# hyye/lio-mapping

Measured on AMD Instinct MI355X. Metric: sliding-window solves/sec, 64-line 130k-pt scans, window=15 (opt_window=5), higher is better.
Workload: dtype f64 (solve) / f32 (features); 1 GPU; HDL-64E outdoor_test_config_64, S_outdoor ray-cast scans, window_size=15 opt_window_size=5, one SolveOptimization per step, clouds resident in HBM; n_lidar_residuals=78236, local_map_points=76752, surf_stack_points=19386, parallelism=1 window

## Files before the change

### lio-mapping_amd/csrc/capi.hip

```cpp
#include <cstring>
#include <new>

#include "../../include/lio_c.h"
#include "../../include/lio_test_hooks.h"
#include "../../include/lio_ext.h"
#include "../../include/lio_full_cloud.h"
#include "../../include/lio_odom_batch.h"
#include "../../include/lio_frontend_batch.h"
#include "../../include/lio_map_batch.h"
#include "est_batch.h"
#include "seg_sort.h"
#include "estimator.h"
#include "rccl_comm.h"
#include "host_init.h"
#include "kf_batch.h"
#include <mutex>
#include <thread>
#include <atomic>
#include <algorithm>

#include "mapping.h"
#include "odometry.h"
#include "pointproc.h"

using namespace lio;

struct lio_pim { std::shared_ptr<Preintegration> p; };
struct lio_map { std::unique_ptr<MappingDev> m; bool borrowed = false; };
struct lio_est { std::unique_ptr<Estimator> e; EstConfig cfg; lio_map map; lio_map_config map_cfg; std::unique_ptr<EstimatorBatch> solo; bool adopted = false; struct lio_est_batch *owner = nullptr; };
struct lio_est_batch {
  std::unique_ptr<EstimatorBatch> b, b2;
  int n1 = 0;
  int parts_opt = 0;
  std::vector<std::pair<std::string, int>> options;
  std::vector<lio_est *> members;
};
static constexpr int kBatchSplitFrom = 96;
struct lio_pp_pool { PointProcessorDev pp; std::mutex mu; unsigned long gen = 0; lio_pp_pool(float lo, float up, int r, const lio_pp_config &c) : pp(lo, up, r, c) {} };
struct lio_pp { std::unique_ptr<PointProcessorDev> pp; std::shared_ptr<lio_pp_pool> pool; int pool_sweep = -1; unsigned long pool_gen = 0; };
struct lio_odom { std::unique_ptr<OdometryDev> o; };

static V3d v3(const double *p) { return V3d(p[0], p[1], p[2]); }
// ... 550 lines not shown
  DBuf<int32_t> idx;
  DBuf<float> sqd, nbr;
  DBuf<float> bounds;
  DBuf<double> gn_partials, gn_sums;
  DBuf<OdomState> gn_state;
  DBuf<KfDesc> gn_kd;
  DBuf<float> gn_rows;
};
static Scratch &scratch() {
  static thread_local Scratch sc;
  if (!sc.s) {
    int nd = 0;
    LIO_HIP(hipGetDeviceCount(&nd));
    if (nd <= 0) throw DeviceError("no HIP device: the product has no CPU path");
    LIO_HIP(hipStreamCreate(&sc.s));
  }
  return sc;
}

int lio_voxel_grid(const float *xyzi, size_t n, float leaf, float *out, size_t *n_out) {
  if ((!xyzi && n) || !out || !n_out || !(leaf > 0)) return LIO_ERR_ARG;
  return guarded([&] {
    Scratch &sc = scratch();
    sc.a.reserve(std::max<size_t>(n, 1));
    if (n) LIO_HIP(hipMemcpyAsync(sc.a.p, xyzi, n * sizeof(float4), hipMemcpyHostToDevice, sc.s));
    size_t m = sc.vox.run(sc.a.p, n, leaf, sc.b, sc.s);
    if (m) LIO_HIP(hipMemcpyAsync(out, sc.b.p, m * sizeof(float4), hipMemcpyDeviceToHost, sc.s));
    LIO_HIP(hipStreamSynchronize(sc.s));
    *n_out = m;
    return LIO_OK;
  });
}

int lio_knn(const float *map, size_t n_map, const float *query, size_t m, int k, float radius_sq, int32_t *idx, float *sqd) {
  if ((!map && n_map) || (!query && m) || !(k == 1 || k == 5) || !idx || !sqd) return LIO_ERR_ARG;
  if (!(radius_sq > 0)) return LIO_ERR_ARG;
  if (m > size_t(INT_MAX) / 8 || n_map > size_t(INT_MAX)) return LIO_ERR_CAPACITY;
  return guarded([&] {
    Scratch &sc = scratch();
    sc.a.reserve(std::max<size_t>(n_map, 1)); sc.b.reserve(std::max<size_t>(m, 1));
    sc.idx.reserve(std::max<size_t>(m * k, 1)); sc.sqd.reserve(std::max<size_t>(m * k, 1));
    if (n_map) LIO_HIP(hipMemcpyAsync(sc.a.p, map, n_map * sizeof(float4), hipMemcpyHostToDevice, sc.s));
    if (m) LIO_HIP(hipMemcpyAsync(sc.b.p, query, m * sizeof(float4), hipMemcpyHostToDevice, sc.s));
    float mn[3], mx[3];
    host_cloud_bounds(map, n_map, mn, mx);
    sc.grid.build(sc.a.p, n_map, mn, mx, knn_cell_edge(radius_sq), sc.s);
    launch_knn(sc.b.p, int(m), k, radius_sq, sc.grid.sorted(), sc.grid.cells(), sc.grid.desc(), sc.idx.p, sc.sqd.p, sc.s);
    if (m) {
      LIO_HIP(hipMemcpyAsync(idx, sc.idx.p, m * k * sizeof(int32_t), hipMemcpyDeviceToHost, sc.s));
      LIO_HIP(hipMemcpyAsync(sqd, sc.sqd.p, m * k * sizeof(float), hipMemcpyDeviceToHost, sc.s));
    }
    LIO_HIP(hipStreamSynchronize(sc.s));
    return LIO_OK;
  });
}

int lio_knn_walk(const float *map, size_t n_map, const float *query, size_t m, float cell, int lanes_per_query, int32_t *idx, float *sqd,
                 float *nbr_xyz) {
  if ((!map && n_map) || (!query && m) || !idx || !sqd || !nbr_xyz || !(cell > 0) || !std::isfinite(cell)) return LIO_ERR_ARG;
  if (!(lanes_per_query == 1 || lanes_per_query == 4 || lanes_per_query == 8)) return LIO_ERR_ARG;
  if (m > size_t(INT_MAX) / 8 || n_map > size_t(INT_MAX)) return LIO_ERR_CAPACITY;
  return guarded([&] {
    Scratch &sc = scratch();
    sc.a.reserve(std::max<size_t>(n_map, 1)); sc.b.reserve(std::max<size_t>(m, 1));
    sc.idx.reserve(std::max<size_t>(m * 5, 1)); sc.sqd.reserve(std::max<size_t>(m * 5, 1)); sc.nbr.reserve(std::max<size_t>(m * 15, 1));
    if (n_map) LIO_HIP(hipMemcpyAsync(sc.a.p, map, n_map * sizeof(float4), hipMemcpyHostToDevice, sc.s));
// ... 920 lines not shown
```

### lio-mapping_amd/csrc/cloud_device.h

```cpp
#pragma once
#include <hip/hip_runtime.h>

#include <cfloat>
#include <climits>

#include "cloud_kernels.h"
#include "hmath.h"

#if defined(__HIPCC__)
namespace lio {

__device__ inline bool finite3(const float4 &p) { return isfinite(p.x) && isfinite(p.y) && isfinite(p.z); }
__device__ inline bool finite3(const Vec3<float> &p) { return isfinite(p.x) && isfinite(p.y) && isfinite(p.z); }


template <bool NORMALISE_CONJ>
__device__ __forceinline__ float4 to_end_point(float4 p, float s, const Quat<float> &qe, const Vec3<float> &te) {
  p.x -= s * te.x; p.y -= s * te.y; p.z -= s * te.z;
  Quat<float> qid;
  Quat<float> qs = slerp(qid, s, qe, FLT_EPSILON);
  Quat<float> qc = conj(qs);
  if (NORMALISE_CONJ) qc = normalized(qc);
  Vec3<float> v = rotate(qc, Vec3<float>(p.x, p.y, p.z));
  v = rotate(qe, v);
// ... 147 lines not shown
                                                     const int *__restrict__ tile_heads, int n, int tile, float4 *__restrict__ out) {
  __shared__ float4 sp[VOX_TILE];
  __shared__ uint32_t sk[VOX_TILE];
  __shared__ int swave[VOX_TILE / 64], sbase[VOX_TILE / 64];
  const int tid = threadIdx.x, lane = tid & 63, wv = tid >> 6;
  const int base_i = tile * VOX_TILE, i = base_i + tid;
  int before = 0;
  for (int b = tid; b < tile; b += VOX_TILE) before += tile_heads[b];
#pragma unroll
  for (int o = 32; o > 0; o >>= 1) before += __shfl_xor(before, o, 64);
  const uint32_t k = i < n ? keys[i] : VOX_KEY_NONE;
  sk[tid] = k;
  if (k != VOX_KEY_NONE) sp[tid] = pts[vals[i]];
  const bool head = vox_is_head(keys, i, k);
  const unsigned long long hb = __ballot(head);
  if (lane == 0) { swave[wv] = __popcll(hb); sbase[wv] = before; }
  __syncthreads();
  int pos = (sbase[0] + sbase[1]) + (sbase[2] + sbase[3]);
  for (int w = 0; w < wv; ++w) pos += swave[w];
  pos += __popcll(hb & ((1ull << lane) - 1ull));
  if (head) {
    float ax = 0, ay = 0, az = 0, ai = 0;
    int e = tid;
    while (e < VOX_TILE && sk[e] == k) { const float4 p = sp[e]; ax += p.x; ay += p.y; az += p.z; ai += p.w; ++e; }
    int cnt = e - tid;
    if (e == VOX_TILE) {
      int g = base_i + VOX_TILE;
      while (g < n && keys[g] == k) { const float4 p = pts[vals[g]]; ax += p.x; ay += p.y; az += p.z; ai += p.w; ++g; ++cnt; }
    }
    const float c = float(cnt);
    out[pos] = make_float4(ax / c, ay / c, az / c, ai / c);
  }
  return VoxSlot{pos, head};
}

__device__ __forceinline__ void clear_valid_block(uint8_t *__restrict__ valid, size_t n) {
  const size_t i = (size_t(blockIdx.x) * VOX_TILE + threadIdx.x) * 16;
  if (i + 16 <= n) *reinterpret_cast<uint4 *>(valid + i) = make_uint4(0, 0, 0, 0);
  else for (size_t k = i; k < n; ++k) valid[k] = 0;
}
__device__ __forceinline__ void odom_state_init(OdomState *__restrict__ st, const float *__restrict__ T, bool converged) {
  static_assert(offsetof(OdomState, T) == 0 && sizeof(OdomState) <= VOX_TILE * 4, "state layout: T first, the rest zero");
  unsigned *o = reinterpret_cast<unsigned *>(st);
  const int nw = int(sizeof(OdomState) / 4);
  if (int(threadIdx.x) < nw) {
    unsigned v = threadIdx.x < 8 ? __float_as_uint(T[threadIdx.x]) : 0u;
    if (converged && threadIdx.x == offsetof(OdomState, converged) / 4) v = 1u;
    o[threadIdx.x] = v;
  }
}


#define FEAT_LPQ 8
#ifndef KNN_BATCH
#define KNN_BATCH 4
#endif
__device__ __forceinline__ unsigned long long knn_key(float d, int idx) {
  return (static_cast<unsigned long long>(__float_as_uint(d)) << 32) | static_cast<unsigned int>(idx);
}
template <int K>
__device__ __forceinline__ void knn_insert(unsigned long long key, int j, unsigned long long (&bk)[K], int (&bj)[K]) {
  if (key < bk[K - 1]) {
    bk[K - 1] = key; bj[K - 1] = j;
#pragma unroll
    for (int k = K - 1; k > 0; --k) {
      const bool sw = bk[k - 1] > bk[k];
// ... 452 lines not shown
```

### lio-mapping_amd/csrc/cloud_kernels.h

```cpp
#pragma once
#include <cmath>
#include <cstdint>

#include "dev.h"
#include "hmath.h"

namespace lio {

struct VoxParams {
  float mn[3], mx[3];
  int minb[3], divb[3];
  int overflow;
  int n_valid;
};

struct Affine3f { float m[12]; };

#define LIO_MAX_FRAMES 32

struct ConcatSeg { const float4 *src; int n; int dst_off; int set_intensity; float intensity; Affine3f tf; int identity; };
struct ConcatArgs { ConcatSeg seg[LIO_MAX_FRAMES]; int nseg; int total; };
void launch_transform_concat(const ConcatArgs &a, float4 *dst, hipStream_t s);

void launch_deskew_to_end(float4 *pts, int n, const float q[4], const float p[3], float time_factor, hipStream_t s, bool keep_intensity = false);
void launch_rigid_map(const float4 *in, int n, const float q[4], const float p[3], float4 *out, hipStream_t s);

void launch_cloud_bounds(const float4 *pts, int n, DBuf<float> &partial, VoxParams *d_out, hipStream_t s);

class VoxelGridDev {
 public:
  size_t run(const float4 *in, size_t n, float leaf, DBuf<float4> &out, hipStream_t s, VoxParams *host_params = nullptr);
  void launch(const float4 *in, size_t n, float leaf, DBuf<float4> &out, hipStream_t s);
  size_t finish(VoxParams *host_params = nullptr);
  void set_host_signal(bool on) { use_signal_ = on; }
  VoxelGridDev() = default;
  VoxelGridDev(const VoxelGridDev &) = delete;
  VoxelGridDev &operator=(const VoxelGridDev &) = delete;

 private:
  const float4 *p_in_ = nullptr; size_t p_n_ = 0; DBuf<float4> *p_out_ = nullptr; hipStream_t p_stream_ = nullptr;
  float p_leaf_ = 0.f;
  void enqueue(bool exact);
  HostBuf<char> h_mail_;
  int *h_count_ = nullptr;
  VoxParams *h_params_ = nullptr;
  DBuf<float> partial_;
  DBuf<VoxParams> params_;
  DBuf<uint32_t> keys_, keys2_, vals_, vals2_;
  DBuf<int> count_, tile_heads_;
  DBuf<char> tmp_;
  unsigned *h_flag_ = nullptr;
  unsigned seq_ = 0;
  HostSignal sig_{};
  bool use_signal_ = true;
};

struct GridDesc {
  int origin[3];
  int dims[3];
  float inv_cell;
  int n_points;
};

inline float knn_cell_edge(float min_match_sq_dis) { return std::sqrt(min_match_sq_dis) * 1.0001f + 1e-6f; }
inline float scan_to_map_cell_edge(float min_match_sq_dis) { return std::sqrt(min_match_sq_dis) * 1.0001f; }
inline void host_cloud_bounds(const float *xyzi, size_t n, float mn[3], float mx[3]) {
  for (int d = 0; d < 3; ++d) { mn[d] = 0.f; mx[d] = 0.f; }
  bool first = true;
  for (size_t i = 0; i < n; ++i) {
    const float *p = xyzi + 4 * i;
    if (!std::isfinite(p[0]) || !std::isfinite(p[1]) || !std::isfinite(p[2])) continue;
    for (int d = 0; d < 3; ++d) {
      if (first || p[d] < mn[d]) mn[d] = p[d];
      if (first || p[d] > mx[d]) mx[d] = p[d];
    }
// ... 131 lines not shown
```

### lio-mapping_amd/csrc/cloud_kernels.hip

```cpp
#include <cstring>
#include <hip/hip_runtime.h>
#include <rocprim/rocprim.hpp>

#include <cfloat>
#include <climits>

#include "cloud_kernels.h"
#include "cloud_device.h"

namespace lio {

__global__ void k_transform_concat(ConcatArgs a, float4 *__restrict__ dst) {
  int gid = blockIdx.x * blockDim.x + threadIdx.x;
  if (gid >= a.total) return;
  int sidx = 0;
  for (int k = 1; k < a.nseg; ++k)
    if (gid >= a.seg[k].dst_off) sidx = k;
  const ConcatSeg &sg = a.seg[sidx];
  int local = gid - sg.dst_off;
  float4 p = sg.src[local];
  float4 o;
  if (sg.identity) {
    o = p;
  } else {
// ... 77 lines not shown
  int i = blockIdx.x * blockDim.x + threadIdx.x;
  if (i >= n) return;
  float4 p = pts[i];
  uint32_t key = VOX_KEY_NONE;
  if (finite3(p)) {
    int i0 = int(floorf(p.x * inv_leaf) - float(vp->minb[0]));
    int i1 = int(floorf(p.y * inv_leaf) - float(vp->minb[1]));
    int i2 = int(floorf(p.z * inv_leaf) - float(vp->minb[2]));
    key = uint32_t(i0 + i1 * vp->divb[0] + i2 * vp->divb[0] * vp->divb[1]);
  }
  keys[i] = key;
  vals[i] = uint32_t(i);
}

__global__ void __launch_bounds__(VOX_TILE) k_vox_keys_abs(const float4 *__restrict__ pts, int n, float inv_leaf, uint32_t *__restrict__ keys,
                                                          uint32_t *__restrict__ vals, float *__restrict__ partial, int *__restrict__ range_overflow) {
  const int i = blockIdx.x * VOX_TILE + threadIdx.x;
  float mn[3] = {FLT_MAX, FLT_MAX, FLT_MAX}, mx[3] = {-FLT_MAX, -FLT_MAX, -FLT_MAX};
  float cnt = 0;
  if (i < n) {
    const float4 p = pts[i];
    uint32_t key = VOX_KEY_NONE;
    if (finite3(p)) {
      cnt = 1.f;
      mn[0] = mx[0] = p.x; mn[1] = mx[1] = p.y; mn[2] = mx[2] = p.z;
      if (!vox_abs_key<10>(p, inv_leaf, key)) *range_overflow = 1;
    }
    keys[i] = key;
    vals[i] = uint32_t(i);
  }
  vox_block_partial(mn, mx, cnt, partial + size_t(blockIdx.x) * 8);
}

__global__ void __launch_bounds__(VOX_TILE) k_vox_tile_heads(const uint32_t *__restrict__ keys, int n, int *__restrict__ tile_heads,
                                                             const float *__restrict__ partial, int npartial, float inv_leaf, VoxParams *__restrict__ params) {
  if (blockIdx.x == gridDim.x - 1) {
    if (npartial <= 0) return;
    VoxParams v;
    if (vox_fold_bounds(partial, npartial, inv_leaf, v)) *params = v;
    return;
  }
  vox_tile_head_count(keys, n, blockIdx.x, tile_heads + blockIdx.x);
}

struct VoxMail { int count; VoxParams params; int range_overflow; };
__global__ void __launch_bounds__(VOX_TILE) k_vox_centroids(const float4 *__restrict__ pts, const uint32_t *__restrict__ keys,
                                                            const uint32_t *__restrict__ vals, const int *__restrict__ tile_heads, int n,
                                                            float4 *__restrict__ out, int *__restrict__ count, const VoxParams *__restrict__ params,
                                                            int *__restrict__ range_overflow, VoxMail *mail, HostSignal sig) {
  const VoxSlot r = vox_centroid_tile(pts, keys, vals, tile_heads, n, blockIdx.x, out);
  if (blockIdx.x == gridDim.x - 1) {
    __shared__ VoxMail smail;
    const int tid = threadIdx.x;
    if (tid == VOX_TILE - 1) {
      const int total = r.pos + (r.head ? 1 : 0);
      *count = total;
      smail.count = total; smail.params = *params; smail.range_overflow = *range_overflow;
      if (sig.flag) *range_overflow = 0;
    }
    if (sig.flag) {
      __syncthreads();
      if (tid < 64) post_host_mail(sig, mail, &smail, int(sizeof(VoxMail) / 4), tid);
    }
  }
}

void launch_cloud_bounds(const float4 *pts, int n, DBuf<float> &partial, VoxParams *d_out, hipStream_t s) {
  const int nb = std::max(1, std::min(cdiv(n, 256), 512));
  partial.reserve(size_t(nb) * 8);
  hipLaunchKernelGGL(k_bounds_partial, dim3(nb), dim3(256), 0, s, pts, n, partial.p);
  hipLaunchKernelGGL(k_bounds_final, dim3(1), dim3(256), 0, s, partial.p, nb, 1.0f, d_out);
  LIO_HIP(hipGetLastError());
}

void VoxelGridDev::launch(const float4 *in, size_t n, float leaf, DBuf<float4> &out, hipStream_t s) {
  p_in_ = in; p_n_ = n; p_out_ = &out; p_stream_ = s; p_leaf_ = leaf;
  if (n == 0) return;
  enqueue(false);
}

void VoxelGridDev::enqueue(bool exact) {
  const float4 *in = p_in_;
  const size_t n = p_n_;
  DBuf<float4> &out = *p_out_;
  hipStream_t s = p_stream_;
  const int ni = int(n);
  const float inv_leaf = 1.0f / p_leaf_;
  const int nkb = cdiv(ni, VOX_TILE);
  partial_.reserve(size_t(std::max(nkb, 512)) * 8);
  params_.reserve(1);
  keys_.reserve(n); keys2_.reserve(n); vals_.reserve(n); vals2_.reserve(n);
  if (count_.cap < 2) { count_.reserve(2); LIO_HIP(hipMemsetAsync(count_.p, 0, count_.cap * sizeof(int), s)); }
  out.reserve(n);
  if (!h_count_) {
    h_mail_.alloc(256, hipHostMallocCoherent, true);
    static_assert(sizeof(VoxMail) <= 128, "mailbox layout");
    h_count_ = reinterpret_cast<int *>(h_mail_.p);
    h_params_ = reinterpret_cast<VoxParams *>(h_count_ + 1);
    h_flag_ = reinterpret_cast<unsigned *>(reinterpret_cast<char *>(h_count_) + 128);
  }
  int *d_range = count_.p + 1;
  if (!use_signal_) LIO_HIP(hipMemsetAsync(d_range, 0, sizeof(int), s));
  int npartial = 0;
  if (exact) {
    const int nb = std::min(cdiv(ni, 256), 512);
    hipLaunchKernelGGL(k_bounds_partial, dim3(nb), dim3(256), 0, s, in, ni, partial_.p);
    hipLaunchKernelGGL(k_bounds_final, dim3(1), dim3(256), 0, s, partial_.p, nb, inv_leaf, params_.p);
    hipLaunchKernelGGL(k_vox_keys, dim3(cdiv(ni, 256)), dim3(256), 0, s, in, ni, inv_leaf, params_.p, keys_.p, vals_.p);
  } else {
    hipLaunchKernelGGL(k_vox_keys_abs, dim3(nkb), dim3(VOX_TILE), 0, s, in, ni, inv_leaf, keys_.p, vals_.p, partial_.p, d_range);
    npartial = nkb;
  }
  size_t tmp_bytes = 0;
  LIO_HIP(rocprim::radix_sort_pairs(nullptr, tmp_bytes, keys_.p, keys2_.p, vals_.p, vals2_.p, n, 0, 32, s));
  tmp_.reserve(tmp_bytes + 256);
  LIO_HIP(rocprim::radix_sort_pairs(tmp_.p, tmp_bytes, keys_.p, keys2_.p, vals_.p, vals2_.p, n, 0, 32, s));
  const int ntiles = cdiv(ni, VOX_TILE);
  tile_heads_.reserve(ntiles);
  hipLaunchKernelGGL(k_vox_tile_heads, dim3(ntiles + 1), dim3(VOX_TILE), 0, s, keys2_.p, ni, tile_heads_.p, partial_.p, npartial, inv_leaf, params_.p);
  sig_ = HostSignal();
  if (use_signal_) { sig_.flag = h_flag_; sig_.seq = ++seq_; }

  hipLaunchKernelGGL(k_vox_centroids, dim3(ntiles), dim3(VOX_TILE), 0, s, in, keys2_.p, vals2_.p, tile_heads_.p, ni, out.p, count_.p, params_.p, d_range,
                     reinterpret_cast<VoxMail *>(h_count_), sig_);
  LIO_HIP(hipGetLastError());
  if (!sig_.flag) {
    VoxMail *m = reinterpret_cast<VoxMail *>(h_count_);
    LIO_HIP(hipMemcpyAsync(&m->count, count_.p, sizeof(int), hipMemcpyDeviceToHost, s));
    LIO_HIP(hipMemcpyAsync(&m->params, params_.p, sizeof(VoxParams), hipMemcpyDeviceToHost, s));
    LIO_HIP(hipMemcpyAsync(&m->range_overflow, d_range, sizeof(int), hipMemcpyDeviceToHost, s));
  }
}

size_t VoxelGridDev::finish(VoxParams *host_params) {
  if (p_n_ == 0) {
    if (host_params) std::memset(host_params, 0, sizeof(*host_params));
    return 0;
  }
  const VoxMail *m = reinterpret_cast<const VoxMail *>(h_count_);
  bool redone = false;
  for (;;) {
    if (sig_.flag) wait_host_signal(sig_, p_stream_);
    else LIO_HIP(hipStreamSynchronize(p_stream_));
    if (m->range_overflow == 1 && !redone) {
      enqueue(true);
      redone = true;
      continue;
    }
    if (redone) LIO_HIP(hipStreamSynchronize(p_stream_));
    break;
  }
  int count = m->count;
  const VoxParams hp = m->params;
  if (hp.overflow) {
    p_out_->reserve(p_n_);
    LIO_HIP(hipMemcpyAsync(p_out_->p, p_in_, p_n_ * sizeof(float4), hipMemcpyDeviceToDevice, p_stream_));
    LIO_HIP(hipStreamSynchronize(p_stream_));
    count = int(p_n_);
  }
  if (host_params) *host_params = hp;
  return size_t(count);
}

size_t VoxelGridDev::run(const float4 *in, size_t n, float leaf, DBuf<float4> &out, hipStream_t s, VoxParams *host_params) {
  launch(in, n, leaf, out, s);
  return finish(host_params);
}

__global__ void k_cell_count(const float4 *__restrict__ pts, int n, GridDesc g, uint32_t *__restrict__ keys, uint32_t *__restrict__ slot,
                             int *__restrict__ cnt) {
  int i = blockIdx.x * blockDim.x + threadIdx.x;
  if (i >= n) return;
  cell_count_point(pts, i, g, keys, slot, cnt);
}

__global__ void k_cell_place(const float4 *__restrict__ pts, const uint32_t *__restrict__ keys, const uint32_t *__restrict__ slot, int n,
                             const int *__restrict__ starts, float4 *__restrict__ sorted, int *__restrict__ cnt) {
  int i = blockIdx.x * blockDim.x + threadIdx.x;
  if (i >= n) return;
  cell_place_point(pts, keys, slot, i, starts, sorted, cnt);
}

void KnnGrid::build(const float4 *pts, size_t n, const float mn[3], const float mx[3], float cell, hipStream_t s) {
  desc_.n_points = int(n);
// ... 445 lines not shown
```

### lio-mapping_amd/lio_amd/capi.py

```python
from __future__ import annotations

import ctypes as C
import os

import numpy as np

_HERE = os.path.dirname(os.path.abspath(__file__))
HIP_LIB_PATH = os.environ.get("LIO_HIP_LIB") or os.path.join(os.path.dirname(_HERE), "csrc", "liblio_hip.so")

c_double_p = C.POINTER(C.c_double)
c_float_p = C.POINTER(C.c_float)
c_int32_p = C.POINTER(C.c_int32)
c_uint8_p = C.POINTER(C.c_uint8)
c_uint16_p = C.POINTER(C.c_uint16)


class TransformF(C.Structure):
    _fields_ = [("q", C.c_float * 4), ("p", C.c_float * 3)]

    @staticmethod
    def make(q_xyzw, p):
        t = TransformF()
        for i in range(4):
            t.q[i] = float(q_xyzw[i])
# ... 251 lines not shown
    "lio_est_map": (C.c_void_p, [C.c_void_p]),
    "lio_est_set_map_refresh": (C.c_int, [C.c_void_p, C.c_int]),
    "lio_est_refresh_map": (C.c_int, [C.c_void_p]),
    "lio_map_get_surround": (C.c_size_t, [C.c_void_p, C.c_float, c_float_p]),
    "lio_est_get_last_map_refresh": (C.c_int, [C.c_void_p, C.POINTER(C.c_int), C.POINTER(TransformF), C.POINTER(C.c_int), C.POINTER(C.c_uint32),
                                               C.POINTER(C.c_int), C.POINTER(C.c_size_t), c_float_p, C.POINTER(C.c_size_t), c_float_p]),
}
_FULL_SIGS = {
    "lio_odom_full_to_end": (C.c_int, [C.c_void_p, c_float_p, C.c_size_t, c_float_p]),
    "lio_map_set_full_cloud": (C.c_int, [C.c_void_p, c_float_p, C.c_size_t]),
    "lio_map_get_full_cloud": (C.c_size_t, [C.c_void_p, c_float_p]),
    "lio_est_set_full_cloud": (C.c_int, [C.c_void_p, C.c_int]),
    "lio_est_get_full_stack": (C.c_size_t, [C.c_void_p, C.c_int, c_float_p, C.POINTER(C.c_int)]),
    "lio_est_get_registered_full": (C.c_int, [C.c_void_p, C.c_int, C.POINTER(TransformF), C.POINTER(C.c_size_t), c_float_p]),
    "lio_est_get_full_transform_es": (C.c_int, [C.c_void_p, C.c_int, C.POINTER(TransformF)]),
    "lio_deskew_to_end": (C.c_int, [c_float_p, C.c_size_t, C.POINTER(TransformF), C.c_float, C.c_int, c_float_p]),
}
FULL_MAP_FRAME, FULL_SENSOR_RAW, FULL_SENSOR_END = 1, 2, 3
_c_float_pp, _c_size_p = C.POINTER(c_float_p), C.POINTER(C.c_size_t)
_ODOM_BATCH_SIGS = {
    "lio_odom_process_batch": (C.c_int, [C.POINTER(C.c_void_p), C.c_int, _c_float_pp, _c_size_p, _c_float_pp, _c_size_p, _c_float_pp, _c_size_p,
                                         _c_float_pp, _c_size_p, C.POINTER(TransformF), C.POINTER(TransformF), c_int32_p, c_int32_p]),
}
ODOM_BATCH_MAX_SENSORS = 1024
_FRONTEND_SIGS = {
    "lio_odom_process_batch_from_pp": (C.c_int, [C.POINTER(C.c_void_p), C.POINTER(C.c_void_p), C.c_int, C.POINTER(TransformF), C.POINTER(TransformF),
                                                 c_int32_p, c_int32_p]),
}
_MAP_BATCH_SIGS = {
    "lio_map_process_batch": (C.c_int, [C.POINTER(C.c_void_p), C.c_int, _c_float_pp, _c_size_p, _c_float_pp, _c_size_p, C.POINTER(TransformF),
                                        C.POINTER(TransformF), c_int32_p, c_int32_p]),
}
MAP_BATCH_MAX_SENSORS = 1024


def _dp(a):
    return None if a is None else a.ctypes.data_as(c_double_p)


def _fp(a):
    return None if a is None else a.ctypes.data_as(c_float_p)


def _f64(a):
    return np.ascontiguousarray(a, dtype=np.float64)


def _f32(a):
    return np.ascontiguousarray(a, dtype=np.float32)


class LioError(RuntimeError):
    pass


def _chk(rc, what):
    if rc != 0:
        raise LioError(f"{what} failed with code {rc}")


class LioLib:
    def __init__(self, path):
        if not os.path.exists(path):
            raise LioError(f"{path} is missing — build it first (python -c 'import __graft_entry__ as g; g.build()')")
        self.path = path
        self.dll = C.CDLL(path)
        for name, (res, args) in _SIGS.items():
            fn = getattr(self.dll, name)
            fn.restype = res
            fn.argtypes = args
        self.missing = []
        for name, (res, args) in _TEST_SIGS.items():
            fn = getattr(self.dll, name, None)
            if fn is None:
                self.missing.append(name)
                continue
            fn.restype = res
            fn.argtypes = args
        self.backend = self.dll.lio_backend().decode()
        self.has_ext = self.backend.startswith("hip")
        if self.has_ext:
            for name, (res, args) in (list(_EXT_SIGS.items()) + list(_FULL_SIGS.items()) + list(_ODOM_BATCH_SIGS.items()) + list(_FRONTEND_SIGS.items())
                                      + list(_MAP_BATCH_SIGS.items())):
                fn = getattr(self.dll, name)
                fn.restype = res
                fn.argtypes = args

    def deskew_to_end(self, xyzi, T_es: TransformF, time_factor=10.0, keep_intensity=False):
        c = _f32(xyzi).reshape(-1, 4)
        out = np.zeros_like(c)
        _chk(self.dll.lio_deskew_to_end(_fp(c), c.shape[0], C.byref(T_es), time_factor, 1 if keep_intensity else 0, _fp(out)), "lio_deskew_to_end")
        return out

    @staticmethod
    def _laser_frames(transforms, pims):
        n = len(transforms)
        T = (TransformF * n)(*[TransformF.make(q, p) for q, p in transforms])
        P = (C.c_void_p * n)(*[(p.h if p is not None else None) for p in pims])
        return n, T, P

    def imu_estimate_extrinsic_rotation(self, transforms, pims, T_lb):
        n, T, P = self._laser_frames(transforms, pims)
        lb = TransformF.make(*T_lb)
        rc = self.dll.lio_imu_estimate_extrinsic_rotation(n, T, P, C.byref(lb))
        if rc < 0:
            raise LioError(f"lio_imu_estimate_extrinsic_rotation -> {rc}")
        return bool(rc), lb.to_np()[0]

    def imu_initialization(self, transforms, pims, T_lb, Bgs=None):
        n, T, P = self._laser_frames(transforms, pims)
        lb = TransformF.make(*T_lb)
        Vs = np.zeros((n, 3))
        bgs = np.zeros((n, 3)) if Bgs is None else _f64(Bgs).reshape(n, 3).copy()
        g, R = np.zeros(3), np.zeros((3, 3))
        rc = self.dll.lio_imu_initialization(n, T, P, C.byref(lb), _dp(Vs), _dp(bgs), _dp(g), _dp(R))
        if rc < 0:
            raise LioError(f"lio_imu_initialization -> {rc}")
        return dict(ok=bool(rc), Vs=Vs, Bgs=bgs, g=g, R_WI=R)

    def dense_spd_solve(self, A, b):
        A, b = _f64(A), _f64(b)
        n = b.shape[0]
        assert A.shape == (n, n)
        x = np.zeros(n)
        _chk(self.dll.lio_dense_spd_solve(_dp(A), _dp(b), n, _dp(x)), "lio_dense_spd_solve")
        return x

    def marginalize_schur(self, A, b, m):
        A, b = _f64(A), _f64(b)
        n = b.shape[0] - m
        assert A.shape == (m + n, m + n)
        J, r, s = np.zeros((n, n)), np.zeros(n), np.zeros(n)
        _chk(self.dll.lio_marginalize_schur(_dp(A), _dp(b), m, n, _dp(J), _dp(r), _dp(s)), "lio_marginalize_schur")
        return J, r, s

    def bench_voxel_grid(self, xyzi, leaf, reps=10):
        xyzi = _f32(xyzi).reshape(-1, 4)
        ms, n_out = C.c_double(0), C.c_size_t(0)
        _chk(self.dll.lio_bench_voxel_grid(_fp(xyzi), xyzi.shape[0], float(leaf), int(reps), C.byref(ms), C.byref(n_out)), "lio_bench_voxel_grid")
        return ms.value, int(n_out.value)

    def seg_sort_pairs(self, keys, values, seg_off, seg_n, bits, passes):
        keys = np.ascontiguousarray(keys, dtype=np.uint32)
        vals = None if values is None else np.ascontiguousarray(values, dtype=np.uint32)
        so, sn = np.ascontiguousarray(seg_off, dtype=np.int32), np.ascontiguousarray(seg_n, dtype=np.int32)
        ko, vo = np.zeros_like(keys), np.zeros_like(keys)
        u32 = C.POINTER(C.c_uint32)
        _chk(self.dll.lio_seg_sort_pairs(keys.ctypes.data_as(u32), vals.ctypes.data_as(u32) if vals is not None else None, keys.shape[0],
                                         so.ctypes.data_as(c_int32_p), sn.ctypes.data_as(c_int32_p), so.shape[0], int(bits), int(passes),
                                         ko.ctypes.data_as(u32), vo.ctypes.data_as(u32)), "lio_seg_sort_pairs")
        return ko, vo

    def voxel_grid(self, xyzi, leaf):
        xyzi = _f32(xyzi).reshape(-1, 4)
        out = np.zeros_like(xyzi)
        n = C.c_size_t(0)
        _chk(self.dll.lio_voxel_grid(_fp(xyzi), xyzi.shape[0], leaf, _fp(out), C.byref(n)), "lio_voxel_grid")
        return out[: n.value].copy()

    def knn(self, map_xyzi, query_xyzi, k, radius_sq=0.0):
        m_ = _f32(map_xyzi).reshape(-1, 4)
        q_ = _f32(query_xyzi).reshape(-1, 4)
        idx = np.zeros((q_.shape[0], k), dtype=np.int32)
        sqd = np.zeros((q_.shape[0], k), dtype=np.float32)
        _chk(
            self.dll.lio_knn(_fp(m_), m_.shape[0], _fp(q_), q_.shape[0], k, radius_sq, idx.ctypes.data_as(c_int32_p), _fp(sqd)), "lio_knn"
        )
        return idx, sqd

    def knn_walk(self, map_xyzi, query_xyzi, cell, lanes_per_query):
        m_ = _f32(map_xyzi).reshape(-1, 4)
        q_ = _f32(query_xyzi).reshape(-1, 4)
        idx = np.zeros((q_.shape[0], 5), dtype=np.int32)
        sqd = np.zeros((q_.shape[0], 5), dtype=np.float32)
        nbr = np.zeros((q_.shape[0], 5, 3), dtype=np.float32)
        _chk(self.dll.lio_knn_walk(_fp(m_), m_.shape[0], _fp(q_), q_.shape[0], float(cell), int(lanes_per_query),
                                   idx.ctypes.data_as(c_int32_p), _fp(sqd), _fp(nbr)), "lio_knn_walk")
        return idx, sqd, nbr

    def fit_five(self, form, nbr_xyz, fifth_sqd, stack_xyzi, T: TransformF, fixed_pz=(0.0, 0.0, 0.0), min_match_sq_dis=1.0, min_plane_dis=0.2):
        s_ = _f32(stack_xyzi).reshape(-1, 4)
        m = s_.shape[0]
        n_ = _f32(nbr_xyz).reshape(m, 5, 3)
        f_ = _f32(fifth_sqd).reshape(m)
# ... 917 lines not shown
```

Baseline: 2159 solves/s.

## Replace voxel-grid radix sort with sample sort and bitonic bucket sorts

Replaces rocprim's full 32-bit radix sort of voxel keys with a custom sample sort for clouds up to about 393k points. Splitters are picked by ranking an oversampled key sample, keys are scattered into fixed-capacity buckets, and each bucket is bitonic-sorted in LDS. Clouds of 4096 points or fewer use a single rank-based kernel. The aim is to cut the launch and pass overhead of the multi-pass library sort. In exchange it adds a bucket-overflow check that falls back to a rerun with the library sort, plus test hooks and path statistics.

```diff
diff --git a/include/lio_vox_sort.h b/include/lio_vox_sort.h
--- /dev/null
+++ b/include/lio_vox_sort.h
@@ -0,0 +1,27 @@
+#ifndef LIO_VOX_SORT_H
+#define LIO_VOX_SORT_H
+
+#include "lio_c.h"
+
+#ifdef __cplusplus
+extern "C" {
+#endif
+
+#define LIO_VOX_SORT_SAMPLE 0
+#define LIO_VOX_SORT_SINGLE 1
+#define LIO_VOX_SORT_LIBRARY 2
+
+#define LIO_VOX_SORT_SINGLE_MAX 4096
+#define LIO_VOX_SORT_BUCKET_CAP 4096
+#define LIO_VOX_SORT_MEAN_BUCKET 384
+#define LIO_VOX_SORT_OVERSAMPLE 8
+#define LIO_VOX_SORT_SAMPLE_MAX (1024 * 384)
+
+int lio_vox_sort_pairs(const uint32_t *keys, size_t n, uint32_t *keys_out, uint32_t *vals_out, int *path_out);
+
+int lio_vox_sort_stats(uint64_t out[3]);
+
+#ifdef __cplusplus
+}
+#endif
+#endif
diff --git a/lio-mapping_amd/csrc/capi.hip b/lio-mapping_amd/csrc/capi.hip
--- a/lio-mapping_amd/csrc/capi.hip
+++ b/lio-mapping_amd/csrc/capi.hip
@@ -8,6 +8,7 @@
 #include "../../include/lio_odom_batch.h"
 #include "../../include/lio_frontend_batch.h"
 #include "../../include/lio_map_batch.h"
+#include "../../include/lio_vox_sort.h"
 #include "est_batch.h"
 #include "seg_sort.h"
 #include "estimator.h"
@@ -624,6 +625,29 @@
   });
 }
 
+static_assert(LIO_VOX_SORT_SAMPLE == VSORT_PATH_SAMPLE && LIO_VOX_SORT_SINGLE == VSORT_PATH_SINGLE && LIO_VOX_SORT_LIBRARY == VSORT_PATH_LIBRARY &&
+              LIO_VOX_SORT_SINGLE_MAX == VSORT_CAP && LIO_VOX_SORT_BUCKET_CAP == VSORT_CAP && LIO_VOX_SORT_MEAN_BUCKET == VSORT_MEAN &&
+              LIO_VOX_SORT_OVERSAMPLE == VSORT_OVERSAMPLE && LIO_VOX_SORT_SAMPLE_MAX == VSORT_MAX_N, "the header states the sizing rule of cloud_kernels.h");
+int lio_vox_sort_pairs(const uint32_t *keys, size_t n, uint32_t *keys_out, uint32_t *vals_out, int *path_out) {
+  if (!keys || n == 0 || !keys_out || !vals_out) return LIO_ERR_ARG;
+  if (n >= size_t(INT_MAX)) return LIO_ERR_CAPACITY;
+  return guarded([&] {
+    Scratch &sc = scratch();
+    const int path = sc.vox.sort_pairs_hook(keys, n, keys_out, vals_out, sc.s);
+    if (path_out) *path_out = path;
+    return LIO_OK;
+  });
+}
+int lio_vox_sort_stats(uint64_t out[3]) {
+  if (!out) return LIO_ERR_ARG;
+  return guarded([&] {
+    unsigned long long c[3];
+    scratch().vox.sort_stats(c);
+    for (int k = 0; k < 3; ++k) out[k] = c[k];
+    return LIO_OK;
+  });
+}
+
 int lio_knn(const float *map, size_t n_map, const float *query, size_t m, int k, float radius_sq, int32_t *idx, float *sqd) {
   if ((!map && n_map) || (!query && m) || !(k == 1 || k == 5) || !idx || !sqd) return LIO_ERR_ARG;
   if (!(radius_sq > 0)) return LIO_ERR_ARG;
diff --git a/lio-mapping_amd/csrc/cloud_device.h b/lio-mapping_amd/csrc/cloud_device.h
--- a/lio-mapping_amd/csrc/cloud_device.h
+++ b/lio-mapping_amd/csrc/cloud_device.h
@@ -203,6 +203,119 @@
     out[pos] = make_float4(ax / c, ay / c, az / c, ai / c);
   }
   return VoxSlot{pos, head};
+}
+
+#define VSORT_THREADS 256
+#define VSORT_SCATTER_THREADS 512
+#define VSORT_SCATTER_ITEMS 2
+
+__device__ __forceinline__ unsigned long long vsort_from_lane(unsigned long long v, int byte_addr) {
+  const uint32_t lo = uint32_t(__builtin_amdgcn_ds_bpermute(byte_addr, int(uint32_t(v))));
+  const uint32_t hi = uint32_t(__builtin_amdgcn_ds_bpermute(byte_addr, int(uint32_t(v >> 32))));
+  return (static_cast<unsigned long long>(hi) << 32) | lo;
+}
+
+template <int E>
+__device__ __forceinline__ void vsort_block(unsigned long long (&v)[E], unsigned long long *__restrict__ lds) {
+  constexpr int P = VSORT_THREADS * E;
+  const int base = int(threadIdx.x) * E, lane = int(threadIdx.x) & 63;
+#pragma unroll 1
+  for (int k = 2; k <= P; k <<= 1) {
+#pragma unroll 1
+    for (int j = k >> 1; j >= 64 * E; j >>= 1) {
+      __syncthreads();
+#pragma unroll
+      for (int e = 0; e < E; ++e) lds[base + e] = v[e];
+      __syncthreads();
+      const bool keep_min = ((base & j) == 0) == ((base & k) == 0);
+#pragma unroll
+      for (int e = 0; e < E; ++e) {
+        const unsigned long long o = lds[(base ^ j) + e];
+        if ((o < v[e]) == keep_min) v[e] = o;
+      }
+    }
+#pragma unroll 1
+    for (int j = min(k >> 1, 32 * E); j >= E; j >>= 1) {
+      const bool keep_min = ((base & j) == 0) == ((base & k) == 0);
+      const int partner = (lane ^ (j / E)) << 2;
+#pragma unroll
+      for (int e = 0; e < E; ++e) {
+        const unsigned long long o = vsort_from_lane(v[e], partner);
+        if ((o < v[e]) == keep_min) v[e] = o;
+      }
+    }
+#pragma unroll
+    for (int j = E / 2; j > 0; j >>= 1) {
+      if (j < k) {
+#pragma unroll
+        for (int e = 0; e < E; ++e) {
+          if ((e & j) == 0) {
+            const bool asc = ((base + e) & k) == 0;
+            const unsigned long long x = v[e], y = v[e | j];
+            if ((x > y) == asc) { v[e] = y; v[e | j] = x; }
+          }
+        }
+      }
+    }
+  }
+}
+
+__device__ __forceinline__ int vsort_items_for(int m) {
+  int E = 1;
+  while (VSORT_THREADS * E < m) E <<= 1;
+  return E;
+}
+
+template <int E>
+__device__ __forceinline__ void vsort_pairs_sort_store(const unsigned long long *__restrict__ src, int m, unsigned long long *__restrict__ lds,
+                                                       uint32_t *__restrict__ keys_out, uint32_t *__restrict__ vals_out, int off) {
+  unsigned long long v[E];
+  const int base = int(threadIdx.x) * E;
+#pragma unroll
+  for (int e = 0; e < E; ++e) v[e] = base + e < m ? src[base + e] : ~0ull;
+  vsort_block<E>(v, lds);
+#pragma unroll
+  for (int e = 0; e < E; ++e)
+    if (base + e < m) { keys_out[off + base + e] = uint32_t(v[e] >> 32); vals_out[off + base + e] = uint32_t(v[e]); }
+}
+#define VSORT_RANK_LANES 16
+__device__ __forceinline__ int vsort_rank_of(const uint32_t *__restrict__ ss, int S, int part, unsigned long long mine) {
+  int rank = 0;
+  const uint4 *ss4 = reinterpret_cast<const uint4 *>(ss);
+  for (int q = part; q < S / 4; q += VSORT_RANK_LANES) {
+    const uint4 k4 = ss4[q];
+    const uint32_t j = uint32_t(q) * 4;
+    rank += ((static_cast<unsigned long long>(k4.x) << 32) | j) < mine;
+    rank += ((static_cast<unsigned long long>(k4.y) << 32) | (j + 1)) < mine;
+    rank += ((static_cast<unsigned long long>(k4.z) << 32) | (j + 2)) < mine;
+    rank += ((static_cast<unsigned long long>(k4.w) << 32) | (j + 3)) < mine;
+  }
+#pragma unroll
+  for (int o = VSORT_RANK_LANES / 2; o > 0; o >>= 1) rank += __shfl_xor(rank, o, 64);
+  return rank;
+}
+
+template <int OVERSAMPLE>
+__device__ __forceinline__ void vsort_pick_splitters(const uint32_t *__restrict__ keys, int n, int NB, uint32_t *__restrict__ ss,
+                                                     uint32_t *__restrict__ splitters) {
+  const int S = OVERSAMPLE * NB;
+  static_assert(OVERSAMPLE % 4 == 0, "the sample is read four keys at a time");
+  const uint32_t q = uint32_t(n) / uint32_t(S), r = uint32_t(n) % uint32_t(S);
+  for (int t = threadIdx.x; t < S; t += VSORT_THREADS) ss[t] = keys[uint32_t(t) * q + (q * uint32_t(S) + (2u * uint32_t(t) + 1u) * r) / (2u * uint32_t(S))];
+  __syncthreads();
+  const int i = blockIdx.x * (VSORT_THREADS / VSORT_RANK_LANES) + int(threadIdx.x) / VSORT_RANK_LANES, part = int(threadIdx.x) % VSORT_RANK_LANES;
+  const unsigned long long mine = i < S ? (static_cast<unsigned long long>(ss[i]) << 32) | uint32_t(i) : 0ull;
+  const int rank = vsort_rank_of(ss, S, part, mine);
+  if (part == 0 && i < S && rank >= OVERSAMPLE && rank % OVERSAMPLE == 0) splitters[rank / OVERSAMPLE - 1] = uint32_t(mine >> 32);
+}
+
+__device__ __forceinline__ int vsort_bucket_of(const uint32_t *__restrict__ spl, int NB, uint32_t key) {
+  int lo = 0, hi = NB - 1;
+  while (lo < hi) {
+    const int mid = (lo + hi) >> 1;
+    if (spl[mid] <= key) lo = mid + 1; else hi = mid;
+  }
+  return lo;
 }
 
 __device__ __forceinline__ void clear_valid_block(uint8_t *__restrict__ valid, size_t n) {
diff --git a/lio-mapping_amd/csrc/cloud_kernels.h b/lio-mapping_amd/csrc/cloud_kernels.h
--- a/lio-mapping_amd/csrc/cloud_kernels.h
+++ b/lio-mapping_amd/csrc/cloud_kernels.h
@@ -27,8 +27,18 @@
 
 void launch_cloud_bounds(const float4 *pts, int n, DBuf<float> &partial, VoxParams *d_out, hipStream_t s);
 
+#define VSORT_CAP 4096
+#define VSORT_MEAN 384
+#define VSORT_OVERSAMPLE 8
+#define VSORT_MAX_BUCKETS 1024
+#define VSORT_MAX_N (VSORT_MAX_BUCKETS * VSORT_MEAN)
+enum VoxSortPath { VSORT_PATH_SAMPLE = 0, VSORT_PATH_SINGLE = 1, VSORT_PATH_LIBRARY = 2 };
+inline int vsort_buckets(size_t n) { return int((n + VSORT_MEAN - 1) / VSORT_MEAN); }
+
 class VoxelGridDev {
  public:
+  void sort_stats(unsigned long long out[3]) const { for (int k = 0; k < 3; ++k) out[k] = n_path_[k]; }
+  int sort_pairs_hook(const uint32_t *keys, size_t n, uint32_t *keys_out, uint32_t *vals_out, hipStream_t s);
   size_t run(const float4 *in, size_t n, float leaf, DBuf<float4> &out, hipStream_t s, VoxParams *host_params = nullptr);
   void launch(const float4 *in, size_t n, float leaf, DBuf<float4> &out, hipStream_t s);
   size_t finish(VoxParams *host_params = nullptr);
@@ -40,7 +50,14 @@
  private:
   const float4 *p_in_ = nullptr; size_t p_n_ = 0; DBuf<float4> *p_out_ = nullptr; hipStream_t p_stream_ = nullptr;
   float p_leaf_ = 0.f;
-  void enqueue(bool exact);
+  void enqueue(bool exact, bool library);
+  void reserve_sort(size_t n, hipStream_t s);
+  int enqueue_sort(size_t n, hipStream_t s, bool library);
+  DBuf<uint32_t> splitters_;
+  DBuf<int> fill_;
+  DBuf<unsigned long long> pairs_;
+  int last_path_ = VSORT_PATH_LIBRARY;
+  unsigned long long n_path_[3] = {0, 0, 0};
   HostBuf<char> h_mail_;
   int *h_count_ = nullptr;
   VoxParams *h_params_ = nullptr;
diff --git a/lio-mapping_amd/csrc/cloud_kernels.hip b/lio-mapping_amd/csrc/cloud_kernels.hip
--- a/lio-mapping_amd/csrc/cloud_kernels.hip
+++ b/lio-mapping_amd/csrc/cloud_kernels.hip
@@ -133,6 +133,96 @@
   vox_block_partial(mn, mx, cnt, partial + size_t(blockIdx.x) * 8);
 }
 
+__global__ void __launch_bounds__(VSORT_THREADS) k_vsort_splitters(const uint32_t *__restrict__ keys, int n, int NB, uint32_t *__restrict__ splitters,
+                                                                  int *__restrict__ fill, int *__restrict__ overflow) {
+  __shared__ __attribute__((aligned(16))) uint32_t ss[VSORT_OVERSAMPLE * VSORT_MAX_BUCKETS];
+  if (blockIdx.x == 0) {
+    for (int b = threadIdx.x; b < NB; b += VSORT_THREADS) fill[b] = 0;
+    if (threadIdx.x == 0) *overflow = 0;
+  }
+  vsort_pick_splitters<VSORT_OVERSAMPLE>(keys, n, NB, ss, splitters);
+}
+
+__global__ void __launch_bounds__(VSORT_SCATTER_THREADS) k_vsort_scatter(const uint32_t *__restrict__ keys, int n, int NB,
+                                                                        const uint32_t *__restrict__ splitters, int *__restrict__ fill,
+                                                                        unsigned long long *__restrict__ pairs, int *__restrict__ overflow) {
+  __shared__ uint32_t sspl[VSORT_MAX_BUCKETS];
+  __shared__ int scnt[VSORT_MAX_BUCKETS], sbase[VSORT_MAX_BUCKETS];
+  const int tid = threadIdx.x;
+  for (int b = tid; b < NB; b += VSORT_SCATTER_THREADS) { scnt[b] = 0; if (b < NB - 1) sspl[b] = splitters[b]; }
+  __syncthreads();
+  uint32_t key[VSORT_SCATTER_ITEMS];
+  int bucket[VSORT_SCATTER_ITEMS], rank[VSORT_SCATTER_ITEMS];
+#pragma unroll
+  for (int r = 0; r < VSORT_SCATTER_ITEMS; ++r) {
+    const int i = (blockIdx.x * VSORT_SCATTER_ITEMS + r) * VSORT_SCATTER_THREADS + tid;
+    bucket[r] = -1;
+    if (i < n) {
+      key[r] = keys[i];
+      bucket[r] = vsort_bucket_of(sspl, NB, key[r]);
+      rank[r] = atomicAdd(&scnt[bucket[r]], 1);
+    }
+  }
+  __syncthreads();
+  for (int b = tid; b < NB; b += VSORT_SCATTER_THREADS) {
+    const int c = scnt[b];
+    if (c > 0) sbase[b] = atomicAdd(&fill[b], c);
+  }
+  __syncthreads();
+#pragma unroll
+  for (int r = 0; r < VSORT_SCATTER_ITEMS; ++r) {
+    if (bucket[r] < 0) continue;
+    const int i = (blockIdx.x * VSORT_SCATTER_ITEMS + r) * VSORT_SCATTER_THREADS + tid;
+    const int pos = sbase[bucket[r]] + rank[r];
+    if (pos < VSORT_CAP) pairs[size_t(bucket[r]) * VSORT_CAP + pos] = (static_cast<unsigned long long>(key[r]) << 32) | uint32_t(i);
+    else *overflow = 1;
+  }
+}
+
+__global__ void __launch_bounds__(VSORT_THREADS) k_vsort_buckets(const unsigned long long *__restrict__ pairs, const int *__restrict__ fill, int NB, int n,
+                                                                const int *__restrict__ overflow, uint32_t *__restrict__ keys_out,
+                                                                uint32_t *__restrict__ vals_out) {
+  __shared__ unsigned long long sp[VSORT_CAP];
+  __shared__ int swave[VSORT_THREADS / 64];
+  const int b = blockIdx.x, tid = threadIdx.x;
+  if (*overflow) {
+    const int chunk = (n + NB - 1) / NB;
+    for (int i = b * chunk + tid; i < min(n, (b + 1) * chunk); i += VSORT_THREADS) keys_out[i] = VOX_KEY_NONE;
+    return;
+  }
+  int before = 0;
+  for (int j = tid; j < b; j += VSORT_THREADS) before += min(fill[j], VSORT_CAP);
+#pragma unroll
+  for (int o = 32; o > 0; o >>= 1) before += __shfl_xor(before, o, 64);
+  if ((tid & 63) == 0) swave[tid >> 6] = before;
+  const int m = min(fill[b], VSORT_CAP);
+  __syncthreads();
+  int off = 0;
+#pragma unroll
+  for (int w = 0; w < VSORT_THREADS / 64; ++w) off += swave[w];
+  const unsigned long long *src = pairs + size_t(b) * VSORT_CAP;
+  switch (vsort_items_for(m)) {
+    case 1: vsort_pairs_sort_store<1>(src, m, sp, keys_out, vals_out, off); break;
+    case 2: vsort_pairs_sort_store<2>(src, m, sp, keys_out, vals_out, off); break;
+    case 4: vsort_pairs_sort_store<4>(src, m, sp, keys_out, vals_out, off); break;
+    case 8: vsort_pairs_sort_store<8>(src, m, sp, keys_out, vals_out, off); break;
+    default: vsort_pairs_sort_store<16>(src, m, sp, keys_out, vals_out, off); break;
+  }
+}
+
+__global__ void __launch_bounds__(VSORT_THREADS) k_vsort_single(const uint32_t *__restrict__ keys, int n, int *__restrict__ overflow,
+                                                               uint32_t *__restrict__ keys_out, uint32_t *__restrict__ vals_out) {
+  __shared__ __attribute__((aligned(16))) uint32_t ss[VSORT_CAP];
+  if (blockIdx.x == 0 && threadIdx.x == 0) *overflow = 0;
+  const int S = (n + 3) & ~3;
+  for (int t = threadIdx.x; t < S; t += VSORT_THREADS) ss[t] = t < n ? keys[t] : VOX_KEY_NONE;
+  __syncthreads();
+  const int i = blockIdx.x * (VSORT_THREADS / VSORT_RANK_LANES) + int(threadIdx.x) / VSORT_RANK_LANES, part = int(threadIdx.x) % VSORT_RANK_LANES;
+  const unsigned long long mine = i < n ? (static_cast<unsigned long long>(ss[i]) << 32) | uint32_t(i) : 0ull;
+  const int rank = vsort_rank_of(ss, S, part, mine);
+  if (part == 0 && i < n) { keys_out[rank] = uint32_t(mine >> 32); vals_out[rank] = uint32_t(i); }
+}
+
 __global__ void __launch_bounds__(VOX_TILE) k_vox_tile_heads(const uint32_t *__restrict__ keys, int n, int *__restrict__ tile_heads,
                                                              const float *__restrict__ partial, int npartial, float inv_leaf, VoxParams *__restrict__ params) {
   if (blockIdx.x == gridDim.x - 1) {
@@ -144,11 +234,12 @@
   vox_tile_head_count(keys, n, blockIdx.x, tile_heads + blockIdx.x);
 }
 
-struct VoxMail { int count; VoxParams params; int range_overflow; };
+struct VoxMail { int count; VoxParams params; int range_overflow; int sort_overflow; };
 __global__ void __launch_bounds__(VOX_TILE) k_vox_centroids(const float4 *__restrict__ pts, const uint32_t *__restrict__ keys,
                                                             const uint32_t *__restrict__ vals, const int *__restrict__ tile_heads, int n,
                                                             float4 *__restrict__ out, int *__restrict__ count, const VoxParams *__restrict__ params,
-                                                            int *__restrict__ range_overflow, VoxMail *mail, HostSignal sig) {
+                                                            int *__restrict__ range_overflow, const int *__restrict__ sort_overflow, VoxMail *mail,
+                                                            HostSignal sig) {
   const VoxSlot r = vox_centroid_tile(pts, keys, vals, tile_heads, n, blockIdx.x, out);
   if (blockIdx.x == gridDim.x - 1) {
     __shared__ VoxMail smail;
@@ -156,7 +247,7 @@
     if (tid == VOX_TILE - 1) {
       const int total = r.pos + (r.head ? 1 : 0);
       *count = total;
-      smail.count = total; smail.params = *params; smail.range_overflow = *range_overflow;
+      smail.count = total; smail.params = *params; smail.range_overflow = *range_overflow; smail.sort_overflow = *sort_overflow;
       if (sig.flag) *range_overflow = 0;
     }
     if (sig.flag) {
@@ -177,10 +268,10 @@
 void VoxelGridDev::launch(const float4 *in, size_t n, float leaf, DBuf<float4> &out, hipStream_t s) {
   p_in_ = in; p_n_ = n; p_out_ = &out; p_stream_ = s; p_leaf_ = leaf;
   if (n == 0) return;
-  enqueue(false);
-}
-
-void VoxelGridDev::enqueue(bool exact) {
+  enqueue(false, false);
+}
+
+void VoxelGridDev::enqueue(bool exact, bool library) {
   const float4 *in = p_in_;
   const size_t n = p_n_;
   DBuf<float4> &out = *p_out_;
@@ -190,8 +281,7 @@
   const int nkb = cdiv(ni, VOX_TILE);
   partial_.reserve(size_t(std::max(nkb, 512)) * 8);
   params_.reserve(1);
-  keys_.reserve(n); keys2_.reserve(n); vals_.reserve(n); vals2_.reserve(n);
-  if (count_.cap < 2) { count_.reserve(2); LIO_HIP(hipMemsetAsync(count_.p, 0, count_.cap * sizeof(int), s)); }
+  reserve_sort(n, s);
   out.reserve(n);
   if (!h_count_) {
     h_mail_.alloc(256, hipHostMallocCoherent, true);
@@ -212,10 +302,7 @@
     hipLaunchKernelGGL(k_vox_keys_abs, dim3(nkb), dim3(VOX_TILE), 0, s, in, ni, inv_leaf, keys_.p, vals_.p, partial_.p, d_range);
     npartial = nkb;
   }
-  size_t tmp_bytes = 0;
-  LIO_HIP(rocprim::radix_sort_pairs(nullptr, tmp_bytes, keys_.p, keys2_.p, vals_.p, vals2_.p, n, 0, 32, s));
-  tmp_.reserve(tmp_bytes + 256);
-  LIO_HIP(rocprim::radix_sort_pairs(tmp_.p, tmp_bytes, keys_.p, keys2_.p, vals_.p, vals2_.p, n, 0, 32, s));
+  last_path_ = enqueue_sort(n, s, library);
   const int ntiles = cdiv(ni, VOX_TILE);
   tile_heads_.reserve(ntiles);
   hipLaunchKernelGGL(k_vox_tile_heads, dim3(ntiles + 1), dim3(VOX_TILE), 0, s, keys2_.p, ni, tile_heads_.p, partial_.p, npartial, inv_leaf, params_.p);
@@ -223,14 +310,63 @@
   if (use_signal_) { sig_.flag = h_flag_; sig_.seq = ++seq_; }
 
   hipLaunchKernelGGL(k_vox_centroids, dim3(ntiles), dim3(VOX_TILE), 0, s, in, keys2_.p, vals2_.p, tile_heads_.p, ni, out.p, count_.p, params_.p, d_range,
-                     reinterpret_cast<VoxMail *>(h_count_), sig_);
+                     count_.p + 2, reinterpret_cast<VoxMail *>(h_count_), sig_);
   LIO_HIP(hipGetLastError());
   if (!sig_.flag) {
     VoxMail *m = reinterpret_cast<VoxMail *>(h_count_);
     LIO_HIP(hipMemcpyAsync(&m->count, count_.p, sizeof(int), hipMemcpyDeviceToHost, s));
     LIO_HIP(hipMemcpyAsync(&m->params, params_.p, sizeof(VoxParams), hipMemcpyDeviceToHost, s));
     LIO_HIP(hipMemcpyAsync(&m->range_overflow, d_range, sizeof(int), hipMemcpyDeviceToHost, s));
-  }
+    LIO_HIP(hipMemcpyAsync(&m->sort_overflow, count_.p + 2, sizeof(int), hipMemcpyDeviceToHost, s));
+  }
+}
+
+void VoxelGridDev::reserve_sort(size_t n, hipStream_t s) {
+  keys_.reserve(n); keys2_.reserve(n); vals_.reserve(n); vals2_.reserve(n);
+  if (count_.cap < 3) { count_.reserve(3); LIO_HIP(hipMemsetAsync(count_.p, 0, count_.cap * sizeof(int), s)); }
+}
+
+int VoxelGridDev::enqueue_sort(size_t n, hipStream_t s, bool library) {
+  const int ni = int(n);
+  int *d_overflow = count_.p + 2;
+  if (library || n > size_t(VSORT_MAX_N)) {
+    LIO_HIP(hipMemsetAsync(d_overflow, 0, sizeof(int), s));
+    size_t tmp_bytes = 0;
+    LIO_HIP(rocprim::radix_sort_pairs(nullptr, tmp_bytes, keys_.p, keys2_.p, vals_.p, vals2_.p, n, 0, 32, s));
+    tmp_.reserve(tmp_bytes + 256);
+    LIO_HIP(rocprim::radix_sort_pairs(tmp_.p, tmp_bytes, keys_.p, keys2_.p, vals_.p, vals2_.p, n, 0, 32, s));
+    return VSORT_PATH_LIBRARY;
+  }
+  if (ni <= VSORT_CAP) {
+    hipLaunchKernelGGL(k_vsort_single, dim3(cdiv(ni, VSORT_THREADS / VSORT_RANK_LANES)), dim3(VSORT_THREADS), 0, s, keys_.p, ni, d_overflow, keys2_.p, vals2_.p);
+    return VSORT_PATH_SINGLE;
+  }
+  const int NB = vsort_buckets(n);
+  splitters_.reserve(NB); fill_.reserve(NB); pairs_.reserve(size_t(NB) * VSORT_CAP);
+  hipLaunchKernelGGL(k_vsort_splitters, dim3(cdiv(VSORT_OVERSAMPLE * NB, VSORT_THREADS / VSORT_RANK_LANES)), dim3(VSORT_THREADS), 0, s, keys_.p, ni, NB,
+                     splitters_.p, fill_.p, d_overflow);
+  hipLaunchKernelGGL(k_vsort_scatter, dim3(cdiv(ni, VSORT_SCATTER_THREADS * VSORT_SCATTER_ITEMS)), dim3(VSORT_SCATTER_THREADS), 0, s, keys_.p, ni, NB,
+                     splitters_.p, fill_.p, pairs_.p, d_overflow);
+  hipLaunchKernelGGL(k_vsort_buckets, dim3(NB), dim3(VSORT_THREADS), 0, s, pairs_.p, fill_.p, NB, ni, d_overflow, keys2_.p, vals2_.p);
+  return VSORT_PATH_SAMPLE;
+}
+
+int VoxelGridDev::sort_pairs_hook(const uint32_t *keys, size_t n, uint32_t *keys_out, uint32_t *vals_out, hipStream_t s) {
+  reserve_sort(n, s);
+  std::vector<uint32_t> iota(n);
+  for (size_t i = 0; i < n; ++i) iota[i] = uint32_t(i);
+  LIO_HIP(hipMemcpyAsync(keys_.p, keys, n * sizeof(uint32_t), hipMemcpyHostToDevice, s));
+  LIO_HIP(hipMemcpyAsync(vals_.p, iota.data(), n * sizeof(uint32_t), hipMemcpyHostToDevice, s));
+  int path = enqueue_sort(n, s, false);
+  LIO_HIP(hipGetLastError());
+  int overflow = 0;
+  LIO_HIP(hipMemcpyAsync(&overflow, count_.p + 2, sizeof(int), hipMemcpyDeviceToHost, s));
+  LIO_HIP(hipStreamSynchronize(s));
+  if (overflow) path = enqueue_sort(n, s, true);
+  LIO_HIP(hipMemcpyAsync(keys_out, keys2_.p, n * sizeof(uint32_t), hipMemcpyDeviceToHost, s));
+  LIO_HIP(hipMemcpyAsync(vals_out, vals2_.p, n * sizeof(uint32_t), hipMemcpyDeviceToHost, s));
+  LIO_HIP(hipStreamSynchronize(s));
+  return path;
 }
 
 size_t VoxelGridDev::finish(VoxParams *host_params) {
@@ -239,18 +375,26 @@
     return 0;
   }
   const VoxMail *m = reinterpret_cast<const VoxMail *>(h_count_);
-  bool redone = false;
+  bool redone = false, exact = false, library = false;
   for (;;) {
     if (sig_.flag) wait_host_signal(sig_, p_stream_);
     else LIO_HIP(hipStreamSynchronize(p_stream_));
-    if (m->range_overflow == 1 && !redone) {
-      enqueue(true);
+    if (m->range_overflow == 1 && !exact) {
+      exact = true;
+      enqueue(exact, library);
       redone = true;
       continue;
     }
+    if (m->sort_overflow == 1 && !library) {
+      library = true;
+      enqueue(exact, library);
+      redone = true;
+      continue;
+    }
     if (redone) LIO_HIP(hipStreamSynchronize(p_stream_));
     break;
   }
+  ++n_path_[last_path_];
   int count = m->count;
   const VoxParams hp = m->params;
   if (hp.overflow) {
diff --git a/lio-mapping_amd/lio_amd/capi.py b/lio-mapping_amd/lio_amd/capi.py
--- a/lio-mapping_amd/lio_amd/capi.py
+++ b/lio-mapping_amd/lio_amd/capi.py
@@ -307,6 +307,13 @@
                                         C.POINTER(TransformF), c_int32_p, c_int32_p]),
 }
 MAP_BATCH_MAX_SENSORS = 1024
+_c_uint32_p = C.POINTER(C.c_uint32)
+_VOX_SORT_SIGS = {
+    "lio_vox_sort_pairs": (C.c_int, [_c_uint32_p, C.c_size_t, _c_uint32_p, _c_uint32_p, C.POINTER(C.c_int)]),
+    "lio_vox_sort_stats": (C.c_int, [C.POINTER(C.c_uint64)]),
+}
+VOX_SORT_SAMPLE, VOX_SORT_SINGLE, VOX_SORT_LIBRARY = 0, 1, 2
+VOX_SORT_SINGLE_MAX, VOX_SORT_BUCKET_CAP, VOX_SORT_MEAN_BUCKET, VOX_SORT_OVERSAMPLE = 4096, 4096, 384, 8
 
 
 def _dp(a):
@@ -360,6 +367,11 @@
                 fn = getattr(self.dll, name)
                 fn.restype = res
                 fn.argtypes = args
+            for name, (res, args) in _VOX_SORT_SIGS.items():
+                fn = getattr(self.dll, name, None)
+                if fn is not None:
+                    fn.restype = res
+                    fn.argtypes = args
 
     def deskew_to_end(self, xyzi, T_es: TransformF, time_factor=10.0, keep_intensity=False):
         c = _f32(xyzi).reshape(-1, 4)
@@ -425,6 +437,18 @@
                                          so.ctypes.data_as(c_int32_p), sn.ctypes.data_as(c_int32_p), so.shape[0], int(bits), int(passes),
                                          ko.ctypes.data_as(u32), vo.ctypes.data_as(u32)), "lio_seg_sort_pairs")
         return ko, vo
+
+    def vox_sort_pairs(self, keys):
+        k = np.ascontiguousarray(keys, dtype=np.uint32).reshape(-1)
+        ko, vo, path = np.zeros_like(k), np.zeros_like(k), C.c_int(-1)
+        _chk(self.dll.lio_vox_sort_pairs(k.ctypes.data_as(_c_uint32_p), k.size, ko.ctypes.data_as(_c_uint32_p), vo.ctypes.data_as(_c_uint32_p),
+                                         C.byref(path)), "lio_vox_sort_pairs")
+        return ko, vo, path.value
+
+    def vox_sort_stats(self):
+        out = (C.c_uint64 * 3)()
+        _chk(self.dll.lio_vox_sort_stats(out), "lio_vox_sort_stats")
+        return tuple(int(v) for v in out)
 
     def voxel_grid(self, xyzi, leaf):
         xyzi = _f32(xyzi).reshape(-1, 4)
```

After: 2303 solves/s (median of 6 runs). 6.7% higher.
